# latentnetworks/vimure

Hardware: AMD Instinct MI355X
Metric: CAVI iterations/sec (L=4 N=2000 M=200 K=2 synthetic, mutuality on) (higher is better)
Workload: dtype f64

## Files before the change

### vimure_amd/csrc/vimure_hip.hip

```cpp
#include "vmr_internal.h"
#include "sweep_sl.h"
#include "sweep_gen.h"
#include "sweep_tiles.h"
#include "create.h"
#include "sample_draw.h"

thread_local std::string g_create_err;

__global__ void k_init_rho(const double* __restrict__ pr, double* __restrict__ rho, double* __restrict__ logpr,
                           size_t n, double eps) {
  for (size_t q = blockIdx.x * (size_t)blockDim.x + threadIdx.x; q < n; q += (size_t)gridDim.x * blockDim.x) {
    double v = pr[q];
    rho[q] = v;
    logpr[q] = log(v + eps);
  }
}

__global__ void k_init_rho_pos(const double* __restrict__ pr, double* __restrict__ rho, double* __restrict__ logpr,
                               const unsigned* __restrict__ perm, size_t T, size_t NS, int L, int K, double eps,
                               const unsigned* __restrict__ rs, int* __restrict__ not_onehot) {
  const size_t n = (size_t)L * T * K;
  bool bad = false;
  for (size_t q = blockIdx.x * (size_t)blockDim.x + threadIdx.x; q < n; q += (size_t)gridDim.x * blockDim.x) {
    const size_t row = q / K, k = q - row * K, l = row / T, pos = row - l * T;
// ... 109 lines not shown
    };
    if (t0 < t1) fetch(t0);
    for (long long tb = t0; tb < t1; tb += 64) {
      uint64_t w[NC];
      double r[K];
#pragma unroll
      for (int c = 0; c < NC; ++c) w[c] = wq[c];
#pragma unroll
      for (int k = 0; k < K; ++k) r[k] = rq[k];
      const bool full = cq == 1u;
      if (tb + 64 < t1) fetch(tb + 64);
      bool any = false;
#pragma unroll
      for (int c = 0; c < NC; ++c) {
        if (c < nc) any = any || (w[c] != 0ull);
      }
#pragma unroll
      for (int k = 0; k < K; ++k) accF[k] += (full && !skip_full) ? r[k] : 0.0;
      uint64_t todo = __ballot(any && !full);
      while (todo) {
        int i = __builtin_ctzll(todo);
        todo &= todo - 1;
        double ri[K];
#pragma unroll
        for (int k = 0; k < K; ++k) ri[k] = readlane_f64(r[k], i);
#pragma unroll
        for (int c = 0; c < NC; ++c) {
          if (c < nc) {
            uint64_t wi = readlane64(w[c], i);
            if (__builtin_amdgcn_inverse_ballot_w64(wi)) {
#pragma unroll
              for (int k = 0; k < K; ++k) acc[c][k] += ri[k];
            }
          }
        }
      }
    }
#pragma unroll
    for (int k = 0; k < K; ++k) {
      double u = wave_sum(accF[k]);
#pragma unroll
      for (int c = 0; c < NC; ++c)
        if (c < nc && (cg + c) * 64 + lane < g.M) acc[c][k] += u;
    }
    if (DET) {
      unsigned long long* outd = detA + ((size_t)l * Wp + cg * 64) * K;
#pragma unroll
      for (int c = 0; c < NC; ++c)
#pragma unroll
        for (int k = 0; k < K; ++k)
          if (c < nc && acc[c][k] != 0.0) atomicAdd(&outd[(c * 64 + lane) * K + k], det_fx(acc[c][k], g.det_sha));
      continue;
    }
    for (int q = threadIdx.x; q < NC * 64 * K; q += TPB) sacc[q] = 0.0;
    __syncthreads();
#pragma unroll
    for (int c = 0; c < NC; ++c)
#pragma unroll
      for (int k = 0; k < K; ++k) atomicAdd(&sacc[(c * 64 + lane) * K + k], acc[c][k]);
    __syncthreads();
    double* out = slotA + (((size_t)l * NSLOT + (gb % NSLOT)) * Wp + cg * 64) * K;
    for (int q = threadIdx.x; q < nc * 64 * K; q += TPB) atomicAdd(&out[q], sacc[q]);
    __syncthreads();
  }
}

template <int K>
__global__ __launch_bounds__(TPB) void k_mask_lists(const unsigned* __restrict__ rq, const unsigned short* __restrict__ Rm,
                                                    const unsigned long long* __restrict__ rbase, const uint8_t* __restrict__ rcls,
                                                    const double* __restrict__ rho, double* __restrict__ slotA, int Gl,
                                                    const unsigned* __restrict__ perm , Geo g) {
  extern __shared__ double As[];
  const int l = blockIdx.x / Gl, gb = blockIdx.x - l * Gl;
  const size_t T = (size_t)g.N * g.N;
  const unsigned* rql = rq + (size_t)l * (T + 1);
  const unsigned short* Rml = Rm + rbase[l];
  const uint8_t* cl = rcls + (size_t)l * T;
  const double* rl = rho + (size_t)l * T * K;
  for (int q = threadIdx.x; q < g.Mp * K; q += TPB) As[q] = 0.0;
  __syncthreads();
  const size_t t0 = (size_t)gb * T / Gl, t1 = (size_t)(gb + 1) * T / Gl;
  const unsigned* pl = perm ? perm + (size_t)l * ((T + 63) / 64) * 64 : nullptr;
  for (size_t p = t0 + threadIdx.x; p < t1; p += TPB) {
    const size_t t = pl ? (size_t)pl[p] : p;
    if (cl[t] != 2) continue;
    const unsigned q0 = rql[t], q1 = rql[t + 1];
    double r[K];
#pragma unroll
    for (int k = 0; k < K; ++k) r[k] = rl[p * K + k];
    for (unsigned q = q0; q < q1; ++q) {
      const int m = Rml[q];
#pragma unroll
      for (int k = 0; k < K; ++k) atomicAdd(&As[m * K + k], r[k]);
    }
  }
  __syncthreads();
  double* out = slotA + ((size_t)l * NSLOT + (gb % NSLOT)) * (size_t)g.W * 64 * K;
  for (int q = threadIdx.x; q < g.M * K; q += TPB) {
    const double v = As[q];
    if (v != 0.0) atomicAdd(&out[q], v);
  }
}

__device__ __forceinline__ double h_fold(double* Hl0, size_t copy_stride, size_t idx) {
  double v[NH];
#pragma unroll
  for (int c = 0; c < NH; ++c) v[c] = Hl0[c * copy_stride + idx];
  double t = 0.0;
#pragma unroll
  for (int c = 0; c < NH; ++c) {
    t += v[c];
    if (c > 0) Hl0[c * copy_stride + idx] = 0.0;
  }
  Hl0[idx] = t;
  return t;
}
__device__ __forceinline__ void h_fold_item(double* Hl0, size_t copy_stride, size_t item, int K, const double* Cl, double* out) {
  double rest = 0.0;
  for (int k = K - 1; k >= 0; --k) {
    double v = h_fold(Hl0, copy_stride, item * K + k);
    if (k > 0) rest += v;
    else if (Cl) { v = Cl[item] - v - rest; Hl0[item * K] = v; }
    out[k] = v;
  }
}
__global__ __launch_bounds__(TPB) void k_h_reduce(double* Hg, const double* Cg, Geo g) {
  const size_t items = (size_t)g.Y * g.Mp, hcs = items * g.K, n = (size_t)g.L * items;
  double tmp[KMAX];
  for (size_t q = (size_t)blockIdx.x * TPB + threadIdx.x; q < n; q += (size_t)gridDim.x * TPB) {
    const size_t l = q / items, it = q - l * items;
    h_fold_item(Hg + l * NH * hcs, hcs, it, g.K, Cg ? Cg + l * items : nullptr, tmp);
  }
}
__global__ __launch_bounds__(TPB) void k_take_counts(double* Hg, double* Cg, Geo g) {
  const size_t items = (size_t)g.Y * g.Mp, hcs = items * g.K, n = (size_t)g.L * items;
  for (size_t q = (size_t)blockIdx.x * TPB + threadIdx.x; q < n; q += (size_t)gridDim.x * TPB) {
    const size_t l = q / items, it = q - l * items;
    double* Hl0 = Hg + l * NH * hcs;
    Cg[q] = h_fold(Hl0, hcs, it * g.K + 1);
    Hl0[it * g.K + 1] = 0.0;
  }
}
template <bool ZERO>
__device__ __forceinline__ double h_sum(double* Hl0, size_t, size_t idx) {
  const double v = Hl0[idx];
  if (ZERO) Hl0[idx] = 0.0;
  return v;
}
__device__ __forceinline__ double h_at(const double* Hl0, size_t, size_t idx) { return Hl0[idx]; }

#ifndef FIN_TPB
#define FIN_TPB 512
#endif
__device__ __forceinline__ double block_sum_fin(double v, double* red ) {
  v = wave_sum(v);
  __syncthreads();
  if ((threadIdx.x & 63) == 0) red[threadIdx.x >> 6] = v;
  __syncthreads();
  double r = 0.0;
  if (threadIdx.x == 0) {
    for (int w = 0; w < FIN_TPB / 64; ++w) r += red[w];
  }
  return r;
}

template <bool det >
__device__ __forceinline__ void fin_gamma_body(double* par, double* Hg, const double* __restrict__ Cg, double* slotA, double* slotF,
                                               double* lutg, double* Fg, double* fin , double* nu_acc,
                                               int nh , int do_phi, int consume, const Geo& g,
                                               const int bx, const int fg = FG_G ) {
  extern __shared__ double dyn[];
  __shared__ double red[16];
  __shared__ double ela_old[KMAX], gla_old[KMAX], fk[KMAX];
  __shared__ double lla_n[KMAX], gla_n[KMAX];
  __shared__ int last;
  const ParOff o = par_off(g.L, g.Mp, g.K);
  const int l = bx / fg, gq = bx - l * fg, K = g.K, Wp = g.W * 64, tid = threadIdx.x;
  const int mper = (g.M + fg - 1) / fg, m0 = gq * mper, m1 = min(g.M, m0 + mper), nm = max(0, m1 - m0);
  double* s1 = dyn;
  double* gthn = dyn + mper;
  double* finl = fin + (size_t)l * (2 * KMAX + 2);
  if (tid < K) {
    double fv[NSLOT], f = 0.0;
#pragma unroll
    for (int sl = 0; sl < NSLOT; ++sl) fv[sl] = slotF[((size_t)l * NSLOT + sl) * K + tid];
#pragma unroll
    for (int sl = 0; sl < NSLOT; ++sl) f += fv[sl];
    fk[tid] = f;
    ela_old[tid] = par[o.p_shp + l * K + tid] / par[o.p_rte + l * K + tid];
    gla_old[tid] = par[o.G_la + l * K + tid];
  }
  for (int m = tid; m < mper; m += FIN_TPB) { s1[m] = 0.0; gthn[m] = 0.0; }
  __syncthreads();
  const double gnu = par[o.sc + SC_G_NU];
  const size_t hcs = (size_t)g.Y * g.Mp * K;
  double* Hl = Hg + (size_t)l * NH * hcs;
  const int items = g.Y * nm;
  const bool phi2 = do_phi && g.mut;
  const bool cached = items <= FIN_TPB;
  double hv[KMAX], p0[KMAX];
#pragma unroll
  for (int k = 0; k < KMAX; ++k) { hv[k] = 0.0; p0[k] = 0.0; }
  const double* Cl = Cg ? Cg + (size_t)l * g.Y * g.Mp : nullptr;
  auto item = [&](int y, int m, double (&h_)[KMAX], bool zero) {
    const size_t base = ((size_t)y * g.Mp + m) * K;
    double rest = 0.0;
#pragma unroll
    for (int k = KMAX - 1; k >= 0; --k) {
      if (k < K) {
        double v[NH], t = 0.0;
#pragma unroll
        for (int c = 0; c < NH; ++c) v[c] = c < nh ? Hl[(size_t)c * hcs + base + k] : 0.0;
#pragma unroll
        for (int c = 0; c < NH; ++c) {
          t += v[c];
          if (zero && c < nh) Hl[(size_t)c * hcs + base + k] = 0.0;
        }
        if (k > 0) rest += t;
        else if (Cl && nh > 1) t = Cl[(size_t)y * g.Mp + m] - t - rest;
        h_[k] = t;
      }
    }
  };
  for (int it = tid; it < items; it += FIN_TPB) {
    const int y = it / nm, m = m0 + (it - y * nm);
    const double gth = par[o.G_th + (size_t)l * g.Mp + m];
    double acc = 0.0;
    item(y, m, hv, consume && (!phi2 || cached));
#pragma unroll
    for (int k = 0; k < KMAX; ++k) {
      if (k < K) {
        acc += (g.mut ? w1_of(gth * gla_old[k], gnu * (double)y) : 1.0) * hv[k];
        if (y == 0) p0[k] += hv[k];
      }
    }
    if (acc != 0.0) {
      if (det) atomicAdd(reinterpret_cast<unsigned long long*>(&s1[m - m0]), det_fx(acc, g.det_sh));
      else atomicAdd(&s1[m - m0], acc);
    }
  }
  __syncthreads();
  if (det) {
    for (int m = tid; m < mper; m += FIN_TPB) s1[m] = det_back(*reinterpret_cast<unsigned long long*>(&s1[m]), g.det_sh);
    __syncthreads();
  }
  double pr[KMAX];
#pragma unroll
  for (int k = 0; k < KMAX; ++k) pr[k] = 0.0;
  for (int mi = tid; mi < nm; mi += FIN_TPB) {
    const int m = m0 + mi;
    const size_t q = (size_t)l * g.Mp + m;
    double A[KMAX], rte = 0.0;
    const double pa_th = par[o.a_th + q], pb_th = par[o.b_th + q];
    for (int k = 0; k < K; ++k) {
      double av[NSLOT], ak = 0.0;
      if (slotA) {
#pragma unroll
        for (int sl = 0; sl < NSLOT; ++sl) av[sl] = slotA[(((size_t)l * NSLOT + sl) * Wp + m) * K + k];
#pragma unroll
        for (int sl = 0; sl < NSLOT; ++sl) {
          ak += av[sl];
          slotA[(((size_t)l * NSLOT + sl) * Wp + m) * K + k] = 0.0;
        }
      }
      ak += fk[k];
      A[k] = ak;
      rte += ela_old[k] * ak;
    }
    double shp = pa_th + s1[mi];
    rte = pb_th + rte;
    par[o.g_shp + q] = shp; par[o.g_rte + q] = rte;
    double e = shp / rte, lg = digamma_pos(shp) - log(rte);
    const double gn = exp(lg);
    par[o.E_th + q] = e; par[o.l_th + q] = lg; par[o.G_th + q] = gn;
    gthn[mi] = gn;
    for (int k = 0; k < K; ++k) pr[k] += e * A[k];
  }
  __syncthreads();
  double ps[KMAX];
#pragma unroll
  for (int k = 0; k < KMAX; ++k) ps[k] = 0.0;
  if (phi2) {
    if (cached) {
      if (tid < items) {
        const int y = tid / nm, mi = tid - y * nm;
        const double gth = gthn[mi];
#pragma unroll
        for (int k = 0; k < KMAX; ++k) if (k < K) ps[k] = w1_of(gth * gla_old[k], gnu * (double)y) * hv[k];
      }
    } else {
      for (int it = tid; it < items; it += FIN_TPB) {
        const int y = it / nm, mi = it - y * nm;
        const double gth = gthn[mi];
        double h2[KMAX];
        item(y, m0 + mi, h2, consume != 0);
        for (int k = 0; k < K; ++k) ps[k] += w1_of(gth * gla_old[k], gnu * (double)y) * h2[k];
      }
    }
  } else if (!g.mut) {
#pragma unroll
    for (int k = 0; k < KMAX; ++k) ps[k] = p0[k];
  }
  for (int k = 0; k < K; ++k) {
    const double v = block_sum_fin(pr[k], red);
    const double w = block_sum_fin(ps[k], red);
    if (tid == 0) {
      if (det) { double* sl_ = fin + (size_t)g.L * (2 * KMAX + 2) + ((size_t)l * FG_G + gq) * 2 * KMAX; sl_[k] = v; sl_[KMAX + k] = w; }
      else { atomicAdd(&finl[k], v); atomicAdd(&finl[KMAX + k], w); }
    }
  }
  asm volatile("s_waitcnt vmcnt(0)" ::: "memory");
  __syncthreads();
  if (tid == 0) {
    if (fg == 1) last = 1;
    else {
      __builtin_amdgcn_fence(__ATOMIC_RELEASE, "agent");
      asm volatile("s_waitcnt vmcnt(0)" ::: "memory");
      const double t = atomicAdd(&finl[2 * KMAX], 1.0);
      last = (t == (double)(fg - 1));
      if (last) __builtin_amdgcn_fence(__ATOMIC_ACQUIRE, "agent");
      asm volatile("s_waitcnt vmcnt(0)" ::: "memory");
    }
  }
  __syncthreads();
  if (!last) return;
  if (tid < K) {
    const int k = tid, q = l * K + k;
    double sr, ss;
    if (det) {
      sr = 0.0; ss = 0.0;
      const double* sl_ = fin + (size_t)g.L * (2 * KMAX + 2) + (size_t)l * FG_G * 2 * KMAX;
      for (int q = 0; q < FG_G; ++q) { sr += __builtin_nontemporal_load(&sl_[q * 2 * KMAX + k]); ss += __builtin_nontemporal_load(&sl_[q * 2 * KMAX + KMAX + k]); }
    } else { sr = atomicAdd(&finl[k], 0.0); ss = atomicAdd(&finl[KMAX + k], 0.0); }
    const double rte = par[o.b_la + q] + sr;
    if (g.mut && !do_phi) {
      par[o.p_rte_pend + q] = rte;
    } else {
      const double shp = par[o.a_la + q] + ss;
      par[o.p_shp + q] = shp; par[o.p_rte + q] = rte;
      if (g.mut) par[o.p_rte_pend + q] = rte;
      const double lg = digamma_pos(shp) - log(rte);
      par[o.E_la + q] = shp / rte; par[o.l_la + q] = lg; par[o.G_la + q] = exp(lg);
      lla_n[k] = lg; gla_n[k] = exp(lg);
    }
  }
  __syncthreads();
  if (tid == 0) { for (int k = 0; k < 2 * KMAX + 1; ++k) finl[k] = 0.0; }
  if (consume && tid < K) {
#pragma unroll
    for (int sl = 0; sl < NSLOT; ++sl) slotF[((size_t)l * NSLOT + sl) * K + tid] = 0.0;
  }
  if (do_phi && Fg) {
    const int all = g.Y * g.Mp;
    double* Fl = Fg + (size_t)l * all * K;
    const double* lthn = par + o.l_th + (size_t)l * g.Mp;
    const double* gthg = par + o.G_th + (size_t)l * g.Mp;
    for (int it = tid; it < all; it += FIN_TPB) {
      const int y = it / g.Mp, m = it - y * g.Mp;
      const double lt = (m < g.M) ? lthn[m] : 0.0, gt = (m < g.M) ? gthg[m] : 0.0;
      for (int k = 0; k < K; ++k)
        Fl[(size_t)it * K + k] = (m < g.M) ? f_entry(g.mut, lt, gt, lla_n[k], gla_n[k], gnu, y) : 0.0;
    }
  }
  const double* Eth = par + o.E_th + (size_t)l * g.Mp;
  for (int q = tid; q < g.W * 256; q += FIN_TPB) {
    int n = q >> 4, e = q & 15;
    double v = 0.0;
    for (int u = 0; u < 4; ++u) {
      int m = n * 4 + u;
      if (((e >> u) & 1) && m < g.Mp) v += Eth[m];
    }
    lutg[(size_t)l * g.W * 256 + q] = v;
  }
  if (nu_acc && do_phi && g.mut && Cl) {
    const double* gthg = par + o.G_th + (size_t)l * g.Mp;
    double c0 = 0.0;
    for (int it = tid; it < g.Y * g.Mp; it += FIN_TPB) {
      const int y = it / g.Mp, m = it - y * g.Mp;
      if (y > 0 && m < g.M) {
        const double z2 = gnu * (double)y, den = gthg[m] * gla_n[0] + z2;
        if (den != 0.0) c0 += (z2 / den) * Cl[it];
      }
    }
    c0 = block_sum_fin(c0, red);
    if (tid == 0) nu_acc[2 + l] = c0;
  }
}
__global__ __launch_bounds__(FIN_TPB) void k_fin_gamma(double* par, double* Hg, const double* __restrict__ Cg, double* slotA, double* slotF,
                                                       double* lutg, double* Fg, double* fin, double* nu_acc, int nh, int do_phi, int consume, Geo g) {
  fin_gamma_body<false>(par, Hg, Cg, slotA, slotF, lutg, Fg, fin, nu_acc, nh, do_phi, consume, g, (int)blockIdx.x);
}
__global__ __launch_bounds__(FIN_TPB) void k_fin_gamma_det(double* par, double* Hg, const double* __restrict__ Cg, double* slotA, double* slotF,
                                                           double* lutg, double* Fg, double* fin, double* nu_acc, int nh, int do_phi, int consume, Geo g) {
  fin_gamma_body<true>(par, Hg, Cg, slotA, slotF, lutg, Fg, fin, nu_acc, nh, do_phi, consume, g, (int)blockIdx.x);
}
struct FinUnit {
  double *par, *Hg; const double* Cg; double *slotA, *slotF, *lutg, *fin_g, *nu_acc, *slotR, *elbo;
  Geo g; int fg_blk0, fr_blk0, fr_nblk;
};
__global__ __launch_bounds__(FIN_TPB) void k_fin_gamma_b(const FinUnit* __restrict__ units, const int* __restrict__ blk_unit, int fg) {
  const FinUnit& u = units[blk_unit[blockIdx.x]];
  fin_gamma_body<false>(u.par, u.Hg, u.Cg, u.slotA, u.slotF, u.lutg, nullptr, u.fin_g, u.nu_acc, NH, 1, 1, u.g, (int)blockIdx.x - u.fg_blk0, fg);
}

__global__ __launch_bounds__(TPB) void k_fin_phi(double* par, const double* __restrict__ Hg, Geo g) {
  __shared__ double red[8];
  __shared__ double gla_old[KMAX];
  const ParOff o = par_off(g.L, g.Mp, g.K);
  const int l = blockIdx.x, K = g.K;
  if ((int)threadIdx.x < K) gla_old[threadIdx.x] = par[o.G_la + l * K + threadIdx.x];
  __syncthreads();
  const double gnu = par[o.sc + SC_G_NU];
  const size_t hcs = (size_t)g.Y * g.Mp * K;
  const double* Hl = Hg + (size_t)l * NH * hcs;
  double ps[KMAX];
  for (int k = 0; k < KMAX; ++k) ps[k] = 0.0;
  for (int m = threadIdx.x; m < g.M; m += TPB) {
    const double gth = par[o.G_th + (size_t)l * g.Mp + m];
    for (int y = 0; y < g.Y; ++y)
      for (int k = 0; k < K; ++k) ps[k] += w1_of(gth * gla_old[k], gnu * (double)y) * h_at(Hl, hcs, ((size_t)y * g.Mp + m) * K + k);
  }
  for (int k = 0; k < K; ++k) {
    double v = block_sum(ps[k], red);
    if (threadIdx.x == 0) {
      const int q = l * K + k;
      double shp = par[o.a_la + q] + v, rte = par[o.p_rte_pend + q];
      par[o.p_shp + q] = shp; par[o.p_rte + q] = rte;
      double lg = digamma_pos(shp) - log(rte);
      par[o.E_la + q] = shp / rte; par[o.l_la + q] = lg; par[o.G_la + q] = exp(lg);
    }
  }
}

__device__ __forceinline__ double gamma_elbo_term(double pa, double pb, double qa, double qb) {
  return lgamma(qa) - pa * log(qb) + (pa - qa) * digamma_pos(qa) + qa * (1.0 - pb / qb);
}

__device__ __forceinline__ void fin_rho_body(double* par, double* Hg, const double* Cg, double* slotR, double* elbo_out,
                                             double* fin, int do_nu, int do_elbo, int fold, int skip_nu , const Geo& g,
                                             const int bx, const int gx, double* slots = nullptr ) {
  __shared__ double red[8];
  __shared__ int last;
  const ParOff o = par_off(g.L, g.Mp, g.K);
  double* sc = par + o.sc;
  const int l = bx / FR_G, gs = bx - l * FR_G;
  double a0 = 0.0, gt = 0.0;
  if (!skip_nu && (g.mut || fold)) {
    const double gnu = sc[SC_G_NU];
    const size_t hcs = (size_t)g.Y * g.Mp * g.K;
    double* Hl = Hg + (size_t)l * (g.gen ? 1 : NH) * hcs;
    const long long items = (long long)g.Y * g.Mp, i0 = (long long)gs * items / FR_G, i1 = (long long)(gs + 1) * items / FR_G;
    for (long long it = i0 + (int)threadIdx.x; it < i1; it += TPB) {
      const int y = (int)(it / g.Mp), m = (int)(it - (long long)y * g.Mp);
      if (m >= g.M || (y == 0 && !fold)) continue;
      const double gth = par[o.G_th + (size_t)l * g.Mp + m], z2 = gnu * (double)y;
      if (fold) {
        double hk[KMAX];
        h_fold_item(Hl, hcs, (size_t)it, g.K, Cg ? Cg + (size_t)l * items : nullptr, hk);
        for (int k = 0; k < g.K; ++k) {
          const double z1 = gth * par[o.G_la + l * g.K + k];
          if (g.mut && y > 0) a0 += (z2 / (z1 + z2)) * hk[k];
        }
      } else if (g.mut && y > 0) {
        for (int k = 0; k < g.K; ++k) {
          const double hv = g.det ? det_back(reinterpret_cast<const unsigned long long*>(Hl)[(size_t)it * g.K + k], g.det_sh) : Hl[(size_t)it * g.K + k];
          if (hv != 0.0) a0 += (z2 / (gth * par[o.G_la + l * g.K + k] + z2)) * hv;
        }
      }
    }
  }
  if (do_elbo) {
    for (int m = gs * TPB + threadIdx.x; m < g.M; m += FR_G * TPB) {
      const size_t q = (size_t)l * g.Mp + m;
      gt += gamma_elbo_term(par[o.a_th + q], par[o.b_th + q], par[o.g_shp + q], par[o.g_rte + q]);
    }
    if (gs == 0) {
      for (int k = threadIdx.x; k < g.K; k += TPB) {
        const int q = l * g.K + k;
        gt += gamma_elbo_term(par[o.a_la + q], par[o.b_la + q], par[o.p_shp + q], par[o.p_rte + q]);
      }
    }
  }
  a0 = block_sum(a0, red);
  gt = block_sum(gt, red);
  if (threadIdx.x == 0) {
    if (slots) { slots[2 * bx] = a0; slots[2 * bx + 1] = gt; __builtin_amdgcn_fence(__ATOMIC_RELEASE, "agent"); }
    else { atomicAdd(&fin[0], a0); atomicAdd(&fin[1], gt); }
    asm volatile("s_waitcnt vmcnt(0)" ::: "memory");
    const double t = atomicAdd(&fin[2], 1.0);
    last = (t == (double)(gx - 1));
  }
  __syncthreads();
  if (!last) return;
  double a1 = 0, a2 = 0, a3 = 0;
  if (g.gen && g.det) {
    if (threadIdx.x == 0) {
      unsigned long long* pi = reinterpret_cast<unsigned long long*>(slotR);
      unsigned long long s[6] = {0ull, 0ull, 0ull, 0ull, 0ull, 0ull};
      for (int q = 0; q < NSLOT; ++q) {
        const int w = q < NSLOT / 2 ? 0 : 3;
        for (int i = 1; i <= 3; ++i) { s[w + i - 1] += pi[q * 4 + i]; pi[q * 4 + i] = 0ull; }
        pi[q * 4] = 0ull;
      }
      a1 = det_back(s[0], g.det_shr) + det_back(s[3], g.det_shr + DET_SH2);
      a2 = det_back(s[1], g.det_shr) + det_back(s[4], g.det_shr + DET_SH2);
      a3 = det_back(s[2], g.det_shr) + det_back(s[5], g.det_shr + DET_SH2);
    }
  } else if (threadIdx.x < NSLOT) {
    double* ps = slotR + (size_t)threadIdx.x * 4;
    a1 = ps[1]; a2 = ps[2]; a3 = ps[3];
    ps[0] = ps[1] = ps[2] = ps[3] = 0.0;
  }
  a1 = block_sum(a1, red); a2 = block_sum(a2, red); a3 = block_sum(a3, red);
  if (threadIdx.x == 0) {
    if (slots) {
      __builtin_amdgcn_fence(__ATOMIC_ACQUIRE, "agent");
      a0 = 0.0; gt = 0.0;
      for (int q = 0; q < gx; ++q) { a0 += __builtin_nontemporal_load(&slots[2 * q]); gt += __builtin_nontemporal_load(&slots[2 * q + 1]); }
    } else {
      a0 = atomicAdd(&fin[0], 0.0);
      gt = atomicAdd(&fin[1], 0.0);
    }
    fin[0] = 0.0; fin[1] = 0.0; fin[2] = 0.0;
    if (do_nu && g.mut) {
      sc[SC_G_NU_STALE] = sc[SC_G_NU];
      sc[SC_NU_SHP] = sc[SC_A_ETA] + a0;
      sc[SC_G_NU] = exp(digamma_pos(sc[SC_NU_SHP]) - log(sc[SC_NU_RTE]));
      sc[SC_E_NU] = sc[SC_NU_SHP] / sc[SC_NU_RTE];
    }
    if (do_elbo) {
      double e = a1 + a2 - sc[SC_E_NU] * a3 + gt;
      e += gamma_elbo_term(sc[SC_A_ETA], sc[SC_B_ETA], sc[SC_NU_SHP], sc[SC_NU_RTE]);
      elbo_out[0] = e;
    }
    if (!skip_nu) elbo_out[1] = a0;
    elbo_out[2] = a1 + a2 + gt;
    elbo_out[3] = a3;
  }
}
// ... 252 lines not shown
  h->h_reduced = true;
  return VMR_OK;
}

static int begin_sum_a(vmr_ctx* h, hipStream_t st) {
  const Geo& g = h->g;
  if (!h->a_zero) HIPCHK(h, hipMemsetAsync(h->slotA, 0, (size_t)g.L * NSLOT * g.W * 64 * g.K * 8, st));
  h->a_zero = false;
  return VMR_OK;
}
__global__ __launch_bounds__(256) void k_det_fold(unsigned long long* __restrict__ d, double* __restrict__ Hg, double* __restrict__ slotA,
                                                 double* __restrict__ slotF, double* __restrict__ slotR, Geo g) {
  const size_t nH = (size_t)g.Y * g.Mp * g.K, nA = (size_t)g.W * 64 * g.K, L = (size_t)g.L, K = (size_t)g.K;
  const size_t tot = L * nH + L * nA + L * K + 4;
  for (size_t q = (size_t)blockIdx.x * 256 + threadIdx.x; q < tot; q += (size_t)gridDim.x * 256) {
    const unsigned long long u = d[q];
    if (u == 0ull) continue;
    d[q] = 0ull;
    if (q < L * nH) { const size_t l = q / nH, i = q - l * nH; Hg[l * NH * nH + i] += det_back(u, g.det_sh); }
    else if (q < L * nH + L * nA) { const size_t r = q - L * nH, l = r / nA, i = r - l * nA; slotA[l * NSLOT * nA + i] += det_back(u, g.det_sha); }
    else if (q < L * nH + L * nA + L * K) { const size_t r = q - L * nH - L * nA, l = r / K, k = r - l * K; slotF[l * NSLOT * K + k] += det_back(u, g.det_sha); }
    else { const size_t r = q - L * nH - L * nA - L * K; slotR[r] += det_back(u, g.det_shr); }
  }
}
static int det_fold(vmr_ctx* h) {
  const Geo& g = h->g;
  if (!g.det) return VMR_OK;
  const size_t tot = (size_t)g.L * g.Y * g.Mp * g.K + (size_t)g.L * g.W * 64 * g.K + (size_t)g.L * g.K + 4;
  hipLaunchKernelGGL(k_det_fold, dim3((unsigned)std::min<size_t>(1024, (tot + 255) / 256)), dim3(256), 0, h->stream, h->det_buf, h->Hg, h->slotA, h->slotF,
                     h->slotR, g);
  HIPCHK(h, hipGetLastError());
  return VMR_OK;
}

static int ensure_rho(vmr_ctx* h) {
  if (!h->rho_stale) return VMR_OK;
  const SlShape shs = sl_shape(h, true, false, false);
  SlArgs as = sl_args(h, shs, 0, 0);
  as.slotF = nullptr; as.slotA = nullptr;
  as.nu_stale = h->g.mut ? 1 : 0;
  int rc = sl_launch(h, 0, shs, as);
  if (rc) return rc;
  HIPCHK(h, hipGetLastError());
  h->rho_stale = false;
  return VMR_OK;
}

int ensure_rho_ext(vmr_ctx* h) { return ensure_rho(h); }

static int launch_hist(vmr_ctx* h, int nu = -1) {
  const Geo& g = h->g;
  if (g.gen) return gen_hist(h);
  { int rce = ensure_rho(h); if (rce) return rce; }
  HIPCHK(h, hipMemsetAsync(h->Hg, 0, (size_t)g.L * NH * g.Y * g.Mp * g.K * 8, h->stream));
  if (h->sparse) {
    HIPCHK(h, hipMemsetAsync(h->slotF, 0, (size_t)g.L * NSLOT * g.K * 8, h->stream));
    h->f_valid = g.fuse_full != 0;
    if (g.ml) { int rc = begin_sum_a(h, h->stream); if (rc) return rc; h->a_valid = true; }
    Prof p(h, VMR_KERNEL_GAMMA_COUNTS);
    const SlShape shs = sl_shape(h, false, false, true);
    SlArgs as = sl_args(h, shs, 1, g.ml);
    if (nu >= 0 && g.mut) { as.nu_acc = h->nu_acc; as.elbo_dev = h->elbo_dev; as.commit_nu = nu; }
    as.det = g.det ? h->det_buf : nullptr;
    int rcs = sl_launch(h, 3, shs, as);
    if (rcs) return rcs;
    HIPCHK(h, hipGetLastError());
    if (g.farl && (rcs = launch_far(h, 0, (nu >= 0 && g.mut) ? nu : -1))) return rcs;
    if (as.h0s) {
      hipLaunchKernelGGL(k_level0_spread, dim3(g.L), dim3(256), 0, h->stream, h->Hg, h->Cg, h->h0s, g);
      HIPCHK(h, hipGetLastError());
    }
    if ((rcs = det_fold(h))) return rcs;
  } else {
    Prof p(h, VMR_KERNEL_GAMMA_COUNTS);
    int rc = tiles_hist(h);
    if (rc) return rc;
  }
  HIPCHK(h, hipGetLastError());
  h->h_valid = true;
  h->h_zero = false;
  h->h_reduced = false;
  return VMR_OK;
}

static int launch_gamma(vmr_ctx* h, bool with_phi) {
  const Geo& g = h->g;
  h->prte_valid = !with_phi;
  if (g.gen) return gen_gamma(h, with_phi);
  if (h->sparse && !h->h_valid) {
    int rc = launch_hist(h);
    if (rc) return rc;
  }
  hipStream_t ms = h->h_valid ? h->stream : h->stream2;
  if (ms != h->stream) {
    HIPCHK(h, hipEventRecord(h->ev_fork, h->stream));
    HIPCHK(h, hipStreamWaitEvent(ms, h->ev_fork, 0));
  }
  const int skip_full = (g.fuse_full && h->f_valid) ? 1 : 0;
  if (skip_full && h->n_partial > 0 && h->rq && h->a_valid) {
  } else if (skip_full && h->n_partial > 0 && h->rq) {
    { int rc = begin_sum_a(h, ms); if (rc) return rc; }
    Prof p(h, VMR_KERNEL_GAMMA_MASK, ms);
    const size_t T_ = (size_t)g.N * g.N;
    int gl = (int)std::min<size_t>(std::max<size_t>(1, (size_t)h->ncu / g.L), (T_ + 4 * TPB - 1) / (4 * TPB));
    const size_t lsm = (size_t)g.Mp * g.K * 8;
    if (lsm > 48 * 1024 && !h->ml_attr) {
      DISPATCH_K(g.K, HIPCHK(h, hipFuncSetAttribute(reinterpret_cast<const void*>(k_mask_lists<KK>),
                                                    hipFuncAttributeMaxDynamicSharedMemorySize, (int)lsm)));
      h->ml_attr = true;
    }
    DISPATCH_K(g.K, hipLaunchKernelGGL((k_mask_lists<KK>), dim3(g.L * gl), dim3(TPB), lsm, ms, h->rq, h->Rm, h->rbase,
                                       h->rcls, h->rho, h->slotA, gl, h->perm, g));
  } else if (!skip_full || h->n_partial > 0) {
    Prof p(h, VMR_KERNEL_GAMMA_MASK, ms);
    dim3 grid(g.L * g.Gm), blk(TPB);
    unsigned long long* detA = g.det ? h->det_buf + (size_t)g.L * g.Y * g.Mp * g.K : nullptr;
#define GMASK(NC_)                                                                                                                              \
  do {                                                                                                                                          \
    if (g.det) { DISPATCH_K(g.K, hipLaunchKernelGGL((k_gamma_mask<KK, NC_, true>), grid, blk, 0, ms, h->Rb, h->rho, h->rcls, h->slotA, skip_full, h->perm, g, detA)); } \
    else { DISPATCH_K(g.K, hipLaunchKernelGGL((k_gamma_mask<KK, NC_, false>), grid, blk, 0, ms, h->Rb, h->rho, h->rcls, h->slotA, skip_full, h->perm, g, detA)); }    \
  } while (0)
    switch (g.W >= 4 ? 4 : g.W) {
      case 1: GMASK(1); break;
      case 2: GMASK(2); break;
      case 3: GMASK(3); break;
      default: GMASK(4); break;
    }
#undef GMASK
    if (g.det) {
      if (ms != h->stream) return fail(h, VMR_ESTATE, "deterministic mask sums beside a statistics pass");
      HIPCHK(h, hipGetLastError());
      int rcd = det_fold(h);
      if (rcd) return rcd;
    }
  }
  if (ms != h->stream) {
    HIPCHK(h, hipEventRecord(h->ev_join, ms));
    int rc = launch_hist(h);
    if (rc) return rc;
    HIPCHK(h, hipStreamWaitEvent(h->stream, h->ev_join, 0));
  } else if (!h->h_valid) {
    int rc = launch_hist(h);
    if (rc) return rc;
  }
  {
    Prof p(h, VMR_KERNEL_FINALIZE);
    const int consume = (with_phi && !g.two_pass) ? 1 : 0;
    const int nh = h->h_reduced ? 1 : NH;
    const size_t fsm = (size_t)2 * ((g.M + FG_G - 1) / FG_G) * 8;
    hipLaunchKernelGGL(g.det ? k_fin_gamma_det : k_fin_gamma, dim3(g.L * FG_G), dim3(FIN_TPB), fsm, h->stream, h->par, h->Hg, h->sparse ? h->Cg : nullptr,
                       (h->sparse && skip_full && h->n_partial == 0) ? nullptr : h->slotA,
                       h->slotF, h->lutg, nullptr, h->fin_g, h->sparse ? h->nu_acc : nullptr, nh,
                       with_phi ? 1 : 0, consume, g);
    h->a_valid = false; h->a_zero = true;
    if (consume) { h->h_valid = false; h->f_valid = false; h->h_zero = true; }
  }
  HIPCHK(h, hipGetLastError());
  return VMR_OK;
}

static int launch_phi(vmr_ctx* h) {
  const Geo& g = h->g;
  if (g.gen) return gen_phi(h);
  if (!g.mut) return VMR_OK;
  if (!h->h_valid) { int rc = launch_hist(h); if (rc) return rc; }
  { int rc = ensure_h_folded(h); if (rc) return rc; }
  {
    Prof p(h, VMR_KERNEL_FINALIZE);
    hipLaunchKernelGGL(k_fin_phi, dim3(g.L), dim3(TPB), 0, h->stream, h->par, h->Hg, g);
  }
  HIPCHK(h, hipGetLastError());
  return VMR_OK;
}

static int launch_rho(vmr_ctx* h, int mode, bool commit_nu, bool raw_nu = false, bool store = true) {
  const Geo& g = h->g;
  if (mode != 2) h->prte_valid = false;
  if (g.gen) return gen_rho(h, mode, commit_nu, raw_nu, [](vmr_ctx* hh, int do_nu, int do_elbo, int skip_nu) { return launch_fin_rho(hh, do_nu, do_elbo, skip_nu); });
  if (h->sparse && g.farl && h->elbo_split && mode == 1) {
    int rc2 = launch_rho(h, 0, commit_nu, raw_nu, true);
    if (rc2) return rc2;
    const SlShape she = sl_shape(h, false, true, false);
    SlArgs ae = sl_args(h, she, 0, 0);
    ae.elbo_cur = commit_nu ? 0 : 1;
    {
      Prof p(h, VMR_KERNEL_ELBO);
      if ((rc2 = sl_launch(h, 2, she, ae))) return rc2;
    }
    HIPCHK(h, hipGetLastError());
    return launch_fin_rho(h, 0, 1, 1);
  }
  size_t sm = shmem_rho(g, mode != 2, mode != 0);
  int rc = VMR_OK;
  if (mode != 2 && !h->h_zero) {
    if (g.fuse_full) HIPCHK(h, hipMemsetAsync(h->slotF, 0, (size_t)g.L * NSLOT * g.K * 8, h->stream));
    if (!g.two_pass) HIPCHK(h, hipMemsetAsync(h->Hg, 0, (size_t)g.L * NH * g.Y * g.Mp * g.K * 8, h->stream));
  }
  if (mode != 2) h->h_zero = false;
  const bool nu_in_pass = h->sparse && g.mut && mode != 2 && (commit_nu || raw_nu);
  if (mode == 2 && (rc = ensure_rho(h))) return rc;
  if (h->sparse) {
    const int do_hist = (mode != 2 && !g.two_pass) ? 1 : 0;
    const int sum_a = (g.ml && do_hist) ? 1 : 0;
    if (mode != 2) h->a_valid = false;
    if (sum_a) { if ((rc = begin_sum_a(h, h->stream))) return rc; h->a_valid = true; }
    const SlShape shs = sl_shape(h, mode != 2, mode != 0, do_hist != 0);
    SlArgs as = sl_args(h, shs, do_hist, sum_a);
    if (nu_in_pass && do_hist) { as.nu_acc = h->nu_acc; as.elbo_dev = h->elbo_dev; as.commit_nu = commit_nu ? 1 : 0; }
    as.det = g.det ? h->det_buf : nullptr;
    const bool lazy = !store && mode == 0 && do_hist && (nu_in_pass ? commit_nu : !g.mut) && g.fuse_full && (h->n_partial == 0 || g.ml) &&
                      !g.farl && !h->opt.always_store_rho;
    {
      Prof p(h, lazy ? VMR_KERNEL_RHO_NOSTORE : mode == 2 ? VMR_KERNEL_ELBO : mode == 1 ? VMR_KERNEL_RHO_ELBO : VMR_KERNEL_RHO);
      if ((rc = sl_launch(h, lazy ? 4 : mode, shs, as))) return rc;
    }
    if (mode != 2) h->rho_stale = lazy;
    if (g.farl && do_hist && (rc = launch_far(h, 0, nu_in_pass ? (commit_nu ? 1 : 0) : -1))) return rc;
    if ((rc = det_fold(h))) return rc;
  } else {
    Prof p(h, mode == 2 ? VMR_KERNEL_ELBO : mode == 1 ? VMR_KERNEL_RHO_ELBO : VMR_KERNEL_RHO);
    if ((rc = tiles_rho(h, mode, sm))) return rc;
  }
  if (mode != 2) {
    h->f_valid = g.fuse_full != 0;
    h->h_valid = !g.two_pass;
    if (!g.two_pass) h->h_reduced = false;
    if (g.two_pass && (rc = launch_hist(h, nu_in_pass ? (commit_nu ? 1 : 0) : -1))) return rc;
  }
  HIPCHK(h, hipGetLastError());
  if (nu_in_pass || (h->sparse && mode != 2 && !g.mut)) {
    if (mode != 0 && (rc = launch_fin_rho(h, 0, 1, 1))) return rc;
  } else if (mode != 0 || commit_nu) {
    if ((rc = launch_fin_rho(h, (mode != 2 && commit_nu) ? 1 : 0, mode != 0 ? 1 : 0))) return rc;
  }
  return VMR_OK;
}

extern "C" {

const char* vmr_version(void) { return VMR_VERSION; }

const char* vmr_last_error(vmr_handle h) { return h ? h->err.c_str() : g_create_err.c_str(); }

int vmr_data_stats(vmr_handle h, double* sum_x, uint8_t* coverage) {
  if (!h) return VMR_EINVAL;
  HIPCHK(h, hipSetDevice(h->device));
  unsigned long long v = 0;
  if (sum_x) HIPCHK(h, hipMemcpyAsync(&v, h->sumx, 8, hipMemcpyDeviceToHost, h->stream));
  if (coverage) HIPCHK(h, hipMemcpyAsync(coverage, h->cov, (size_t)h->g.L * h->g.N * h->g.N, hipMemcpyDeviceToHost, h->stream));
  HIPCHK(h, hipStreamSynchronize(h->stream));
  if (sum_x) *sum_x = (double)v;
  return VMR_OK;
}

static int upload_lm(vmr_ctx* h, size_t off, const double* src, double pad) {
  const Geo& g = h->g;
  std::vector<double> buf((size_t)g.L * g.Mp, pad);
  for (int l = 0; l < g.L; ++l) memcpy(&buf[(size_t)l * g.Mp], src + (size_t)l * g.M, (size_t)g.M * 8);
  HIPCHK(h, hipMemcpyAsync(h->par + off, buf.data(), buf.size() * 8, hipMemcpyHostToDevice, h->stream));
  HIPCHK(h, hipStreamSynchronize(h->stream));
  return VMR_OK;
}
static int h2d(vmr_ctx* h, void* dst, const void* src, size_t n) {
  HIPCHK(h, hipMemcpyAsync(dst, src, n, hipMemcpyHostToDevice, h->stream));
  return VMR_OK;
}
static int d2h(vmr_ctx* h, void* dst, const void* src, size_t n) {
  HIPCHK(h, hipMemcpyAsync(dst, src, n, hipMemcpyDeviceToHost, h->stream));
  return VMR_OK;
}

int vmr_set_priors(vmr_handle h, const double* alpha_theta, const double* beta_theta, const double* alpha_lambda,
                   const double* beta_lambda, double alpha_eta, double beta_eta) {
  if (!h || !alpha_theta || !beta_theta || !alpha_lambda || !beta_lambda) return fail(h, VMR_EINVAL, "NULL prior array");
  HIPCHK(h, hipSetDevice(h->device));
  const Geo& g = h->g;
  ParOff o = par_off(g.L, g.Mp, g.K);
  int rc;
  if ((rc = upload_lm(h, o.a_th, alpha_theta, 1.0))) return rc;
  if ((rc = upload_lm(h, o.b_th, beta_theta, 1.0))) return rc;
  if ((rc = h2d(h, h->par + o.a_la, alpha_lambda, (size_t)g.L * g.K * 8))) return rc;
  if ((rc = h2d(h, h->par + o.b_la, beta_lambda, (size_t)g.L * g.K * 8))) return rc;
  double ab[2] = {alpha_eta, beta_eta};
  if ((rc = h2d(h, h->par + o.sc + SC_A_ETA, ab, 16))) return rc;
  HIPCHK(h, hipStreamSynchronize(h->stream));
  h->have_priors = true;
  return VMR_OK;
}

static void drop_graphs(vmr_ctx* h);
int vmr_set_state(vmr_handle h, const double* gamma_shp, const double* gamma_rte, const double* phi_shp,
                  const double* phi_rte, double nu_shp, double nu_rte, const double* pr_rho, int pr_rho_on_device) {
  if (!h || !gamma_shp || !gamma_rte || !phi_shp || !phi_rte || !pr_rho) return fail(h, VMR_EINVAL, "NULL state array");
  if (!h->have_priors) return fail(h, VMR_ESTATE, "vmr_set_priors must be called before vmr_set_state");
  HIPCHK(h, hipSetDevice(h->device));
  const Geo& g = h->g;
  ParOff o = par_off(g.L, g.Mp, g.K);
  int rc;
  if ((rc = upload_lm(h, o.g_shp, gamma_shp, 1.0))) return rc;
  if ((rc = upload_lm(h, o.g_rte, gamma_rte, 1.0))) return rc;
  if ((rc = h2d(h, h->par + o.p_shp, phi_shp, (size_t)g.L * g.K * 8))) return rc;
  if ((rc = h2d(h, h->par + o.p_rte, phi_rte, (size_t)g.L * g.K * 8))) return rc;
  double nu[2] = {nu_shp, nu_rte};
  if ((rc = h2d(h, h->par + o.sc + SC_NU_SHP, nu, 16))) return rc;
  const size_t n = (size_t)g.L * g.N * g.N * g.K;
  const double* src = pr_rho;
// ... 791 lines not shown
```

Baseline: 6268.

## Shorten finalize-gamma tail: merged reductions, prefetch, LDS theta cache

```diff
diff --git a/vimure_amd/csrc/vimure_hip.hip b/vimure_amd/csrc/vimure_hip.hip
--- a/vimure_amd/csrc/vimure_hip.hip
+++ b/vimure_amd/csrc/vimure_hip.hip
@@ -285,6 +285,7 @@
 #ifndef FIN_TPB
 #define FIN_TPB 512
 #endif
+#define FIN_LM 1024
 __device__ __forceinline__ double block_sum_fin(double v, double* red ) {
   v = wave_sum(v);
   __syncthreads();
@@ -297,15 +298,24 @@
   return r;
 }
 
+#ifdef FIN_DEBUG
+#define FIN_NSTAMP 12
+#define FIN_DBG_WG 1024
+__device__ unsigned long long fin_dbg_t[FIN_DBG_WG * FIN_NSTAMP];
+#define FIN_STAMP(i) do { if (threadIdx.x == 0 && bx < FIN_DBG_WG) fin_dbg_t[bx * FIN_NSTAMP + (i)] = wall_clock64(); } while (0)
+#else
+#define FIN_STAMP(i)
+#endif
 template <bool det >
 __device__ __forceinline__ void fin_gamma_body(double* par, double* Hg, const double* __restrict__ Cg, double* slotA, double* slotF,
                                                double* lutg, double* Fg, double* fin , double* nu_acc,
                                                int nh , int do_phi, int consume, const Geo& g,
                                                const int bx, const int fg = FG_G ) {
   extern __shared__ double dyn[];
-  __shared__ double red[16];
+  __shared__ double red[(FIN_TPB / 64) * 2 * KMAX];
   __shared__ double ela_old[KMAX], gla_old[KMAX], fk[KMAX];
   __shared__ double lla_n[KMAX], gla_n[KMAX];
+  __shared__ double thL[2 * FIN_LM];
   __shared__ int last;
   const ParOff o = par_off(g.L, g.Mp, g.K);
   const int l = bx / fg, gq = bx - l * fg, K = g.K, Wp = g.W * 64, tid = threadIdx.x;
@@ -313,6 +323,10 @@
   double* s1 = dyn;
   double* gthn = dyn + mper;
   double* finl = fin + (size_t)l * (2 * KMAX + 2);
+#ifdef FIN_DEBUG
+  if (tid == 0 && bx < FIN_DBG_WG) for (int i = 8; i < FIN_NSTAMP; ++i) fin_dbg_t[bx * FIN_NSTAMP + i] = 0;
+#endif
+  FIN_STAMP(0);
   if (tid < K) {
     double fv[NSLOT], f = 0.0;
 #pragma unroll
@@ -325,6 +339,7 @@
   }
   for (int m = tid; m < mper; m += FIN_TPB) { s1[m] = 0.0; gthn[m] = 0.0; }
   __syncthreads();
+  FIN_STAMP(1);
   const double gnu = par[o.sc + SC_G_NU];
   const size_t hcs = (size_t)g.Y * g.Mp * K;
   double* Hl = Hg + (size_t)l * NH * hcs;
@@ -373,10 +388,23 @@
     }
   }
   __syncthreads();
+  FIN_STAMP(2);
   if (det) {
     for (int m = tid; m < mper; m += FIN_TPB) s1[m] = det_back(*reinterpret_cast<unsigned long long*>(&s1[m]), g.det_sh);
     __syncthreads();
   }
+  const int kk = tid < K ? tid : 0;
+  const double pa_la = par[o.a_la + l * K + kk], pb_la = par[o.b_la + l * K + kk];
+  constexpr int NCP = 4;
+  const bool nu_c = nu_acc && do_phi && g.mut && Cl;
+  const bool c_held = nu_c && g.Y * g.Mp <= NCP * FIN_TPB;
+  double cpre[NCP];
+#pragma unroll
+  for (int j = 0; j < NCP; ++j) {
+    const int it = tid + j * FIN_TPB;
+    cpre[j] = (c_held && it < g.Y * g.Mp) ? Cl[it] : 0.0;
+  }
+  auto publish = [](double* p, double v) { __hip_atomic_store(p, v, __ATOMIC_RELAXED, __HIP_MEMORY_SCOPE_AGENT); };
   double pr[KMAX];
 #pragma unroll
   for (int k = 0; k < KMAX; ++k) pr[k] = 0.0;
@@ -405,11 +433,12 @@
     par[o.g_shp + q] = shp; par[o.g_rte + q] = rte;
     double e = shp / rte, lg = digamma_pos(shp) - log(rte);
     const double gn = exp(lg);
-    par[o.E_th + q] = e; par[o.l_th + q] = lg; par[o.G_th + q] = gn;
+    publish(&par[o.E_th + q], e); publish(&par[o.l_th + q], lg); publish(&par[o.G_th + q], gn);
     gthn[mi] = gn;
     for (int k = 0; k < K; ++k) pr[k] += e * A[k];
   }
   __syncthreads();
+  FIN_STAMP(3);
   double ps[KMAX];
 #pragma unroll
   for (int k = 0; k < KMAX; ++k) ps[k] = 0.0;
@@ -434,42 +463,59 @@
 #pragma unroll
     for (int k = 0; k < KMAX; ++k) ps[k] = p0[k];
   }
-  for (int k = 0; k < K; ++k) {
-    const double v = block_sum_fin(pr[k], red);
-    const double w = block_sum_fin(ps[k], red);
-    if (tid == 0) {
-      if (det) { double* sl_ = fin + (size_t)g.L * (2 * KMAX + 2) + ((size_t)l * FG_G + gq) * 2 * KMAX; sl_[k] = v; sl_[KMAX + k] = w; }
-      else { atomicAdd(&finl[k], v); atomicAdd(&finl[KMAX + k], w); }
-    }
-  }
+  {
+    const int wv = tid >> 6;
+    for (int k = 0; k < K; ++k) {
+      const double v = wave_sum(pr[k]), w = wave_sum(ps[k]);
+      if ((tid & 63) == 0) { red[wv * 2 * KMAX + k] = v; red[wv * 2 * KMAX + KMAX + k] = w; }
+    }
+    __syncthreads();
+    if (tid < 2 * K) {
+      const int q = tid < K ? tid : KMAX + (tid - K);
+      double r = 0.0;
+      for (int w = 0; w < FIN_TPB / 64; ++w) r += red[w * 2 * KMAX + q];
+      if (det) publish(fin + (size_t)g.L * (2 * KMAX + 2) + ((size_t)l * FG_G + gq) * 2 * KMAX + q, r);
+      else atomicAdd(&finl[q], r);
+    }
+  }
+  FIN_STAMP(4);
   asm volatile("s_waitcnt vmcnt(0)" ::: "memory");
   __syncthreads();
+  FIN_STAMP(5);
   if (tid == 0) {
     if (fg == 1) last = 1;
     else {
-      __builtin_amdgcn_fence(__ATOMIC_RELEASE, "agent");
-      asm volatile("s_waitcnt vmcnt(0)" ::: "memory");
+      FIN_STAMP(6);
       const double t = atomicAdd(&finl[2 * KMAX], 1.0);
       last = (t == (double)(fg - 1));
+      FIN_STAMP(7);
       if (last) __builtin_amdgcn_fence(__ATOMIC_ACQUIRE, "agent");
       asm volatile("s_waitcnt vmcnt(0)" ::: "memory");
     }
   }
   __syncthreads();
   if (!last) return;
+  FIN_STAMP(8);
+  double sr = 0.0, ss = 0.0;
+  if (tid < K) {
+    if (det) {
+      const double* sl_ = fin + (size_t)g.L * (2 * KMAX + 2) + (size_t)l * FG_G * 2 * KMAX;
+      for (int q = 0; q < FG_G; ++q) { sr += __builtin_nontemporal_load(&sl_[q * 2 * KMAX + tid]); ss += __builtin_nontemporal_load(&sl_[q * 2 * KMAX + KMAX + tid]); }
+    } else { sr = atomicAdd(&finl[tid], 0.0); ss = atomicAdd(&finl[KMAX + tid], 0.0); }
+  }
+  const bool th_lds = g.Mp <= FIN_LM;
+  const double* Eth = par + o.E_th + (size_t)l * g.Mp;
+  const double* gthg = par + o.G_th + (size_t)l * g.Mp;
+  if (th_lds) {
+    for (int m = tid; m < g.Mp; m += FIN_TPB) { const double e = Eth[m], gt = gthg[m]; thL[m] = e; thL[FIN_LM + m] = gt; }
+  }
   if (tid < K) {
     const int k = tid, q = l * K + k;
-    double sr, ss;
-    if (det) {
-      sr = 0.0; ss = 0.0;
-      const double* sl_ = fin + (size_t)g.L * (2 * KMAX + 2) + (size_t)l * FG_G * 2 * KMAX;
-      for (int q = 0; q < FG_G; ++q) { sr += __builtin_nontemporal_load(&sl_[q * 2 * KMAX + k]); ss += __builtin_nontemporal_load(&sl_[q * 2 * KMAX + KMAX + k]); }
-    } else { sr = atomicAdd(&finl[k], 0.0); ss = atomicAdd(&finl[KMAX + k], 0.0); }
-    const double rte = par[o.b_la + q] + sr;
+    const double rte = pb_la + sr;
     if (g.mut && !do_phi) {
       par[o.p_rte_pend + q] = rte;
     } else {
-      const double shp = par[o.a_la + q] + ss;
+      const double shp = pa_la + ss;
       par[o.p_shp + q] = shp; par[o.p_rte + q] = rte;
       if (g.mut) par[o.p_rte_pend + q] = rte;
       const double lg = digamma_pos(shp) - log(rte);
@@ -478,6 +524,7 @@
     }
   }
   __syncthreads();
+  FIN_STAMP(9);
   if (tid == 0) { for (int k = 0; k < 2 * KMAX + 1; ++k) finl[k] = 0.0; }
   if (consume && tid < K) {
 #pragma unroll
@@ -487,37 +534,42 @@
     const int all = g.Y * g.Mp;
     double* Fl = Fg + (size_t)l * all * K;
     const double* lthn = par + o.l_th + (size_t)l * g.Mp;
-    const double* gthg = par + o.G_th + (size_t)l * g.Mp;
     for (int it = tid; it < all; it += FIN_TPB) {
       const int y = it / g.Mp, m = it - y * g.Mp;
-      const double lt = (m < g.M) ? lthn[m] : 0.0, gt = (m < g.M) ? gthg[m] : 0.0;
+      const double lt = (m < g.M) ? lthn[m] : 0.0, gt = (m < g.M) ? (th_lds ? thL[FIN_LM + m] : gthg[m]) : 0.0;
       for (int k = 0; k < K; ++k)
         Fl[(size_t)it * K + k] = (m < g.M) ? f_entry(g.mut, lt, gt, lla_n[k], gla_n[k], gnu, y) : 0.0;
     }
   }
-  const double* Eth = par + o.E_th + (size_t)l * g.Mp;
   for (int q = tid; q < g.W * 256; q += FIN_TPB) {
     int n = q >> 4, e = q & 15;
     double v = 0.0;
     for (int u = 0; u < 4; ++u) {
       int m = n * 4 + u;
-      if (((e >> u) & 1) && m < g.Mp) v += Eth[m];
+      if (((e >> u) & 1) && m < g.Mp) v += th_lds ? thL[m] : Eth[m];
     }
     lutg[(size_t)l * g.W * 256 + q] = v;
   }
-  if (nu_acc && do_phi && g.mut && Cl) {
-    const double* gthg = par + o.G_th + (size_t)l * g.Mp;
+  FIN_STAMP(10);
+  if (nu_c) {
     double c0 = 0.0;
-    for (int it = tid; it < g.Y * g.Mp; it += FIN_TPB) {
+    auto term = [&](int it, double c) {
       const int y = it / g.Mp, m = it - y * g.Mp;
       if (y > 0 && m < g.M) {
-        const double z2 = gnu * (double)y, den = gthg[m] * gla_n[0] + z2;
-        if (den != 0.0) c0 += (z2 / den) * Cl[it];
+        const double z2 = gnu * (double)y, den = (th_lds ? thL[FIN_LM + m] : gthg[m]) * gla_n[0] + z2;
+        if (den != 0.0) c0 += (z2 / den) * c;
       }
+    };
+    if (c_held) {
+#pragma unroll
+      for (int j = 0; j < NCP; ++j) { const int it = tid + j * FIN_TPB; if (it < g.Y * g.Mp) term(it, cpre[j]); }
+    } else {
+      for (int it = tid; it < g.Y * g.Mp; it += FIN_TPB) term(it, Cl[it]);
     }
     c0 = block_sum_fin(c0, red);
     if (tid == 0) nu_acc[2 + l] = c0;
   }
+  FIN_STAMP(11);
 }
 __global__ __launch_bounds__(FIN_TPB) void k_fin_gamma(double* par, double* Hg, const double* __restrict__ Cg, double* slotA, double* slotF,
                                                        double* lutg, double* Fg, double* fin, double* nu_acc, int nh, int do_phi, int consume, Geo g) {
@@ -1076,6 +1128,15 @@
                        (h->sparse && skip_full && h->n_partial == 0) ? nullptr : h->slotA,
                        h->slotF, h->lutg, nullptr, h->fin_g, h->sparse ? h->nu_acc : nullptr, nh,
                        with_phi ? 1 : 0, consume, g);
+#ifdef FIN_DEBUG
+    if (const char* fn = h->opt.debug_times[0] ? h->opt.debug_times : nullptr) {
+      static unsigned long long hb[FIN_DBG_WG * FIN_NSTAMP];
+      const unsigned long long nb = (unsigned long long)min(g.L * FG_G, FIN_DBG_WG), hd[3] = {nb, FIN_NSTAMP, FG_G};
+      HIPCHK(h, hipStreamSynchronize(h->stream));
+      HIPCHK(h, hipMemcpyFromSymbol(hb, HIP_SYMBOL(fin_dbg_t), nb * FIN_NSTAMP * 8));
+      if (FILE* f = fopen(fn, "ab")) { fwrite(hd, 8, 3, f); fwrite(hb, 8, nb * FIN_NSTAMP, f); fclose(f); }
+    }
+#endif
     h->a_valid = false; h->a_zero = true;
     if (consume) { h->h_valid = false; h->f_valid = false; h->h_zero = true; }
   }
```

After: 6265. Within noise of the previous version (-0.0%).
